# facebookresearch/detectron2

Measured on NVIDIA H100. Metric: Mask R-CNN R50-FPN training hot-path images/sec (custom-op path fwd+bwd, 2 images/GPU), higher is better.
Workload: dtype f32

## Files before the change

detectron2_b200/csrc/deform_conv_tc.cu:

```cuda
#include <algorithm>
#include <cstdlib>
#include <type_traits>

#include "common.cuh"
#include "deform_conv_tc.cuh"
#include "tc_common.cuh"

using namespace d2b_tc;

namespace {

constexpr int kWorkerWarps = 16;
constexpr int kWorkers = kWorkerWarps * 32;
constexpr int kThreads = kWorkers + 128;
constexpr int kLaunchRegs = (65536 / kThreads) & ~7;
constexpr int kWorkerRegs = 112, kSideRegs = 24;
static_assert(kWorkers * kWorkerRegs + (kThreads - kWorkers) * kSideRegs <= kThreads * kLaunchRegs,
              "register budget exceeds the launch allocation");
constexpr int kMaxBN = 128;
constexpr int kRowsPerHalf = 128 / (2 * kWorkerWarps);
constexpr int kTile = 16384;
constexpr int kMaxSmem = 227 * 1024;
constexpr int kGcolPitch = 132;

struct TC {
  int N, Cin, H, W, Cout, kh, kw, sh, sw, ph, pw, dh, dw, G, DG, Ho, Wo, cpg, opg, cpdg, KK, HoWo;
  int pack, SG, cps, ops, cbs, U;
  int tiles_img;
  int stages_img;
  int MC;
  int nks;
  long long off_bs, mask_bs;
  int mask_sigmoid;
};

struct Epi {
  const float* scale;
  const float* shift;
  int relu;
};

struct K1P { int BN, noct, goct, nkp, ksplit, S, tap_bytes, stage_bytes, red; };
struct K2P { int mper, msplit, tap_bytes; };
struct K3P { int BN, noct, sper, nsplit, S, stage_bytes; };

inline size_t align256(size_t v) { return (v + 255) & ~(size_t)255; }

bool make_tc(const d2b_dcn_params* p, TC& d) {
  if (!p) return false;
  d.N = p->N; d.Cin = p->Cin; d.H = p->H; d.W = p->W; d.Cout = p->Cout; d.kh = p->kh; d.kw = p->kw;
  d.sh = p->stride_h; d.sw = p->stride_w; d.ph = p->pad_h; d.pw = p->pad_w; d.dh = p->dil_h; d.dw = p->dil_w;
  d.G = p->groups; d.DG = p->deformable_groups;
  if (d.N < 0 || d.Cin <= 0 || d.H <= 0 || d.W <= 0 || d.Cout <= 0 || d.kh <= 0 || d.kw <= 0 || d.sh <= 0 || d.sw <= 0 ||
      d.ph < 0 || d.pw < 0 || d.dh <= 0 || d.dw <= 0 || d.G <= 0 || d.DG <= 0)
    return false;
  if (d.Cin % d.G || d.Cout % d.G || d.Cin % d.DG) return false;
  d.Ho = (d.H + 2 * d.ph - (d.dh * (d.kh - 1) + 1)) / d.sh + 1;
  d.Wo = (d.W + 2 * d.pw - (d.dw * (d.kw - 1) + 1)) / d.sw + 1;
  if (d.Ho <= 0 || d.Wo <= 0) return false;
  d.cpg = d.Cin / d.G; d.opg = d.Cout / d.G; d.cpdg = d.Cin / d.DG; d.KK = d.kh * d.kw; d.HoWo = d.Ho * d.Wo;
  if (d.cpg >= 64) {
    if (d.cpg % 64) return false;
    d.pack = 1;
  } else {
    if (d.cpg != 16 && d.cpg != 32) return false;
    d.pack = 64 / d.cpg;
    if (d.G % d.pack) return false;
  }
  if (d.cpdg % 64) return false;
  d.SG = d.G / d.pack; d.cps = d.cpg * d.pack; d.ops = d.opg * d.pack; d.cbs = d.cps / 64; d.U = d.KK * d.cbs;
  if (d.ops % 16) return false;
  if (d.KK > 49) return false;
  if ((long long)d.H * d.W * d.Cin >= (1LL << 29)) return false;
  if ((long long)d.HoWo * d.Cout >= (1LL << 31) || (long long)d.Cout * d.cpg * d.KK >= (1LL << 31)) return false;
  d.tiles_img = d2b_cdiv(d.HoWo, 128);
  d.stages_img = d2b_cdiv(d.HoWo, 64);
  d.MC = (d.U + 1) / 2;
  d.nks = d.ops / 64;
  if ((long long)d.N * d.tiles_img > 0x7fffffffLL) return false;
  d.off_bs = (long long)d.DG * 2 * d.KK * d.HoWo;
  d.mask_bs = (long long)d.DG * d.KK * d.HoWo;
  d.mask_sigmoid = 0;
  return true;
}

const float* use_fused_offset_mask(TC& d, const float* offset_mask) {
  d.off_bs = d.mask_bs = (long long)d.DG * 3 * d.KK * d.HoWo;
  d.mask_sigmoid = 1;
  return offset_mask + (size_t)d.DG * 2 * d.KK * d.HoWo;
}

int largest_tile(int n) {
  for (int t = kMaxBN; t >= 16; t >>= 1)
    if (n % t == 0) return t;
  return 0;
}

int best_split(long long base, int work, int max_split, int overhead) {
  int best = 1;
  long long best_cost = -1;
  for (int s = 1; s <= max_split; ++s) {
    const int per = d2b_cdiv(work, s);
    const int parts = d2b_cdiv(work, per);
    const long long cost = (long long)d2b_cdiv(base * parts, d2b_num_sms()) * (per + overhead);
    if (best_cost < 0 || cost < best_cost) {
      best_cost = cost;
      best = parts;
    }
  }
  return best;
}

bool plan_k1(const TC& d, K1P& k, bool colfed = false) {
  k.BN = largest_tile(d.ops);
  if (k.BN < 16) return false;
  k.noct = d.ops / k.BN;
  k.goct = colfed ? 1 : k.noct;
  const int base = d.N * d.tiles_img * d.SG * k.goct;
  k.ksplit = best_split(base, d.KK, d.KK, 1);
  k.nkp = d2b_cdiv(d.KK, k.ksplit);
  k.ksplit = d2b_cdiv(d.KK, k.nkp);
  k.red = k.ksplit > 1;
  const int ndg = d.DG == 1 ? 1 : std::min(d.DG, d2b_cdiv(d.cps, d.cpdg) + 1);
  k.tap_bytes = ndg * k.nkp * 128 * 16;
  k.stage_bytes = 2 * kTile + 2 * k.BN * 128;
  k.S = 3;
  while (k.S > 1 && k.S * k.stage_bytes + k.tap_bytes + 1024 + 128 > kMaxSmem) --k.S;
  return k.S >= 2;
}

bool plan_k1c(const TC& d, K1P& k1, K1P& kc) {
  const long long base = (long long)d.N * d.tiles_img * d.SG * (k1.noct - 1);
  if (k1.goct != 1 || k1.noct < 2 || (long long)d.N * d.tiles_img * (k1.noct - 1) > 0x7fffffffLL) return false;
  kc = k1;
  kc.goct = k1.noct - 1;
  kc.ksplit = best_split(base, d.KK, d.KK, 1);
  kc.nkp = d2b_cdiv(d.KK, kc.ksplit);
  kc.ksplit = d2b_cdiv(d.KK, kc.nkp);
  kc.tap_bytes = 0;
  kc.S = 3;
  while (kc.S > 1 && kc.S * kc.stage_bytes + 1024 + 128 > kMaxSmem) --kc.S;
  if (kc.S < 2) return false;
  k1.red = kc.red = k1.ksplit > 1 || kc.ksplit > 1;
  return true;
}

bool plan_k2(const TC& d, K2P& k) {
  if (d.ops % 64) return false;
  const int base = d.N * d.tiles_img * d.SG;
  k.msplit = best_split(base, d.MC, d.MC, 1);
  k.mper = d2b_cdiv(d.MC, k.msplit);
  k.msplit = d2b_cdiv(d.MC, k.mper);
  const int nkp = std::min(d.KK, (2 * k.mper + d.cbs - 1) / d.cbs + 1);
  const int ndg = d.DG == 1 ? 1 : std::min(d.DG, d2b_cdiv(d.cps, d.cpdg) + 1);
  k.tap_bytes = ndg * nkp * 128 * 16;
  return 2 * 4 * kTile + 128 * kGcolPitch * 4 + k.tap_bytes + 1024 + 128 <= kMaxSmem;
}

bool plan_k3(const TC& d, K3P& k) {
  if (d.ops % 64) return false;
  k.BN = largest_tile(d.ops);
  k.noct = d.ops / k.BN;
  const int units = d.MC * d.SG * k.noct;
  const int total = d.N * d.stages_img;
  k.nsplit = best_split(units, total, std::min(total, 4 * d2b_num_sms()), 3);
  k.sper = d2b_cdiv(total, k.nsplit);
  k.nsplit = d2b_cdiv(total, k.sper);
  k.stage_bytes = 2 * kTile + 2 * k.BN * 128;
  k.S = 3;
  while (k.S > 1 && k.S * k.stage_bytes + 4096 + 1024 + 128 > kMaxSmem) --k.S;
  return k.S >= 2;
}

struct Carve {
  size_t total = 0;
  size_t add(size_t bytes) {
    const size_t at = total;
    total += align256(bytes);
    return at;
  }
};

struct FwdPlan {
  TC d;
  K1P k1, kc;
  bool colfed;
  int split;
  size_t wt, x, total;
  size_t cols_bytes;
};

bool plan_fwd(const d2b_dcn_params* p, int precision, int x_nhwc, bool cols, FwdPlan& P) {
  if (!make_tc(p, P.d) || !plan_k1(P.d, P.k1)) return false;
  const TC& d = P.d;
  Carve ws;
  P.wt = ws.add((size_t)d.SG * P.k1.noct * d.U * 2 * P.k1.BN * 128);
  P.x = ws.add(x_nhwc ? 0 : sizeof(float) * (size_t)d.N * d.H * d.W * d.Cin);
  P.total = ws.total;
  P.cols_bytes = (size_t)d.N * d.tiles_img * d.SG * d.U * (size_t)(precision == 1 ? 2 : 1) * kTile;
  P.split = precision == 1 ? 1 : 0;
  P.colfed = false;
  K1P k1;
  if (cols && P.k1.noct > 1 && plan_k1(d, k1, true) && plan_k1c(d, k1, P.kc)) {
    P.k1 = k1;
    P.colfed = true;
  }
  return true;
}

struct BwdPlan {
  TC d;
  K2P k2;
  K3P k3;
  int split;
  size_t x, gx, gt_px, wt, gt_oc, gw, gw_bytes, total;
};

bool plan_bwd(const d2b_dcn_params* p, int precision, int x_nhwc, int need_data, int need_weight, BwdPlan& P) {
  if (!make_tc(p, P.d) || !plan_k2(P.d, P.k2) || !plan_k3(P.d, P.k3)) return false;
  const TC& d = P.d;
  const size_t xbytes = sizeof(float) * (size_t)d.N * d.H * d.W * d.Cin;
  P.gw_bytes = sizeof(float) * (size_t)d.SG * d.MC * 128 * d.ops;
  Carve ws;
  P.x = ws.add(x_nhwc ? 0 : xbytes);
  P.gx = ws.add(need_data && !x_nhwc ? xbytes : 0);
  P.gt_px = ws.add(need_data ? (size_t)d.N * d.tiles_img * d.SG * d.nks * 2 * kTile : 0);
  P.wt = ws.add(need_data ? (size_t)d.SG * d.MC * d.nks * 2 * kTile : 0);
  P.gt_oc = ws.add(need_weight ? (size_t)d.N * d.stages_img * d.SG * P.k3.noct * 2 * P.k3.BN * 128 : 0);
  P.gw = ws.add(need_weight ? P.gw_bytes : 0);
  P.total = ws.total;
  P.split = precision == 1 ? 1 : 0;
  return true;
}

struct TapRaw {
  float oh, ow, m;
};

__device__ __forceinline__ TapRaw tap_loads(const TC& d, const float* __restrict__ offset, const float* __restrict__ mask,
                                            int b, int dg, int kp, int p) {
  TapRaw r = {0.f, 0.f, 1.f};
  if (p < d.HoWo) {
    const size_t ob = (size_t)b * d.off_bs + ((size_t)dg * 2 * d.KK) * d.HoWo;
    r.oh = __ldg(offset + ob + (size_t)(2 * kp) * d.HoWo + p);
    r.ow = __ldg(offset + ob + (size_t)(2 * kp + 1) * d.HoWo + p);
    if (mask) r.m = __ldg(mask + (size_t)b * d.mask_bs + ((size_t)dg * d.KK + kp) * d.HoWo + p);
  }
  return r;
}

__device__ __forceinline__ int4 tap_finish(const TC& d, const TapRaw& r, bool has_mask, int kp, int p) {
  int4 t = make_int4(0, 0, 0, 0);
  if (p < d.HoWo) {
    const int ho = p / d.Wo, wo = p - ho * d.Wo;
    const int ki = kp / d.kw, kj = kp - ki * d.kw;
    const float hf = (float)(ho * d.sh - d.ph + ki * d.dh) + r.oh;
    const float wf = (float)(wo * d.sw - d.pw + kj * d.dw) + r.ow;
    float m = r.m;
    if (has_mask && d.mask_sigmoid) m = 1.f / (1.f + expf(-m));
    if (hf > -1.f && wf > -1.f && hf < (float)d.H && wf < (float)d.W) {
      const float hfl = floorf(hf), wfl = floorf(wf);
      const int hl = (int)hfl, wl = (int)wfl;
      const bool t0 = hl >= 0, t1 = hl + 1 <= d.H - 1, l0 = wl >= 0, l1 = wl + 1 <= d.W - 1;
      const int flags = (t0 && l0 ? 1 : 0) | (t0 && l1 ? 2 : 0) | (t1 && l0 ? 4 : 0) | (t1 && l1 ? 8 : 0);
      t.x = ((hl * d.W + wl + d.W + 1) << 4) | flags;
      t.y = __float_as_int(hf - hfl);
      t.z = __float_as_int(wf - wfl);
      t.w = __float_as_int(m);
    }
  }
  return t;
}

__device__ __forceinline__ int4 make_tap(const TC& d, const float* __restrict__ offset, const float* __restrict__ mask,
                                         int b, int dg, int kp, int p) {
  return tap_finish(d, tap_loads(d, offset, mask, b, dg, kp, p), mask != nullptr, kp, p);
}

struct Taps4 {
  float4 v0, v1, v2, v3;
};

__device__ __forceinline__ void load_corners(const float* __restrict__ xcb, uint32_t Cin, uint32_t rs, int code, Taps4& t) {
  const float* __restrict__ p = xcb + (uint32_t)(code >> 4) * Cin;
  const float4 z = make_float4(0.f, 0.f, 0.f, 0.f);
  t.v0 = (code & 1) ? __ldg(reinterpret_cast<const float4*>(p)) : z;
  t.v1 = (code & 2) ? __ldg(reinterpret_cast<const float4*>(p + Cin)) : z;
  t.v2 = (code & 4) ? __ldg(reinterpret_cast<const float4*>(p + rs)) : z;
  t.v3 = (code & 8) ? __ldg(reinterpret_cast<const float4*>(p + (rs + Cin))) : z;
}

__device__ __forceinline__ void interp4(const Taps4& t, float w0, float w1, float w2, float w3, float (&v)[4]) {
  const F2 z = f2_pack(0.f, 0.f), p0 = f2_pack(w0, w0), p1 = f2_pack(w1, w1), p2 = f2_pack(w2, w2), p3 = f2_pack(w3, w3);
  F2 a = f2_fma(p0, f2_pack(t.v0.x, t.v0.y), z), b = f2_fma(p0, f2_pack(t.v0.z, t.v0.w), z);
  a = f2_fma(p1, f2_pack(t.v1.x, t.v1.y), a);
  b = f2_fma(p1, f2_pack(t.v1.z, t.v1.w), b);
  a = f2_fma(p2, f2_pack(t.v2.x, t.v2.y), a);
  b = f2_fma(p2, f2_pack(t.v2.z, t.v2.w), b);
  a = f2_fma(p3, f2_pack(t.v3.x, t.v3.y), a);
  b = f2_fma(p3, f2_pack(t.v3.z, t.v3.w), b);
  f2_unpack(a, v[0], v[1]);
  f2_unpack(b, v[2], v[3]);
}

__device__ __forceinline__ void gather_store(const Taps4& t, int4 tap, uint8_t* a_hi, uint8_t* a_lo, uint32_t off,
                                             bool split) {
  const float lh = __int_as_float(tap.y), lw = __int_as_float(tap.z), m = __int_as_float(tap.w);
  const float hh = 1.f - lh, hw = 1.f - lw;
  float v[4];
// ... 99 lines not shown
    }
  }
  __syncthreads();
  if (warp < kWorkerWarps) reg_alloc<kWorkerRegs>();
  else reg_dealloc<kSideRegs>();

  if (warp < kWorkerWarps) {
    const int half = lane >> 4, q = lane & 15;
    const float* __restrict__ ximg = xh + (size_t)b * d.H * d.W * d.Cin - (size_t)(d.W + 1) * d.Cin;
    const uint32_t ucin = (uint32_t)d.Cin, urs = (uint32_t)(d.W * d.Cin);
    float acc[BN / 4];
#pragma unroll
    for (int i = 0; i < BN / 4; ++i) acc[i] = 0.f;
    int kpl = 0, cb = 0;
    auto stage = [&](int t) {
      const int s = t % k.S;
      const uint32_t par = (uint32_t)((t / k.S) & 1);
      const int cbase = sg * d.cps + cb * 64;
      const int4* __restrict__ tp = taps + ((cbase / d.cpdg - dg0) * nkp + kpl) * 128;
      const float* __restrict__ xc = ximg + cbase + q * 4;
      uint8_t* a_hi = smem + s * k.stage_bytes;
      uint8_t* a_lo = a_hi + kTile;
      mbar_wait(&empty_bar[s], par ^ 1u);
      {
        int4 tap[kRowsPerHalf];
        Taps4 c[kRowsPerHalf];
#pragma unroll
        for (int j = 0; j < kRowsPerHalf; ++j) tap[j] = tp[warp * 2 * kRowsPerHalf + j * 2 + half];
#pragma unroll
        for (int j = 0; j < kRowsPerHalf; ++j) load_corners(xc, ucin, urs, tap[j].x, c[j]);
#pragma unroll
        for (int j = 0; j < kRowsPerHalf; ++j) {
          const uint32_t r = (uint32_t)(warp * 2 * kRowsPerHalf + j * 2 + half);
          gather_store(c[j], tap[j], a_hi, a_lo, swz128(r, (uint32_t)(q >> 1)) + (uint32_t)(q & 1) * 8u, split != 0);
        }
      }
      fence_proxy_async();
      __syncwarp();
      if (lane == 0) mbar_arrive(&full_bar[s]);
      mbar_wait(&full_bar[s], par);
      const uint32_t sa = smem_u32(a_hi), sb = sa + 2 * kTile;
      mma_stage<BN, 0>(acc, sa, sa + kTile, sb, sb + (uint32_t)BN * 128u, split);
      if (++cb == d.cbs) { cb = 0; ++kpl; }
    };
    stage(0);
    for (int t = 1; t < nt; ++t) {
      stage(t);
      wgmma_wait<1>();
      __syncwarp();
      if (lane == 0) mbar_arrive(&empty_bar[(t - 1) % k.S]);
    }
    wgmma_wait<0>();
    fwd_epilogue<BN>(acc, ep, d, k, out, b, p0, sg * d.ops + oct * k.BN);
  } else if (warp == kWorkerWarps) {
    if (lane == 0) {
      const uint32_t bytes = (uint32_t)(split ? 2 : 1) * (uint32_t)k.BN * 128u;
      for (int t = 0; t < nt; ++t) {
        const int s = t % k.S;
        const uint32_t par = (uint32_t)((t / k.S) & 1);
        mbar_wait(&empty_bar[s], par ^ 1u);
        const size_t tile = ((size_t)(sg * k.noct + oct) * d.U + (size_t)kp0 * d.cbs + t);
        mbar_arrive_expect_tx(&full_bar[s], bytes);
        bulk_g2s(smem + s * k.stage_bytes + 2 * kTile, wt + tile * (size_t)(2 * k.BN * 128), bytes, &full_bar[s]);
      }
    }
  } else if (warp == kWorkerWarps + 1) {
    if (saving && lane == 0) {
      const uint32_t tile_bytes = (uint32_t)(split ? 2 : 1) * (uint32_t)kTile;
      for (int t = 0; t < nt; ++t) {
        const int s = t % k.S;
        const uint32_t par = (uint32_t)((t / k.S) & 1);
        mbar_wait(&full_bar[s], par);
        const size_t tile = ((size_t)blockIdx.x * d.SG + sg) * d.U + (size_t)kp0 * d.cbs + t;
        bulk_s2g(cols + tile * tile_bytes, smem + s * k.stage_bytes, tile_bytes);
        bulk_commit();
        bulk_wait_read0();
        mbar_arrive(&empty_bar[s]);
      }
      bulk_wait0();
    }
  }
}

template <int BN>
__global__ void __launch_bounds__(kThreads, 1) dcn_fwd_cols_kernel(const uint8_t* __restrict__ cols,
                                                                   const uint8_t* __restrict__ wt, const Epi ep, const TC d,
                                                                   const K1P k, const int split, float* __restrict__ out) {
  extern __shared__ uint8_t smem_raw[];
  uint8_t* smem = smem_raw + ((1024u - (smem_u32(smem_raw) & 1023u)) & 1023u);
  uint64_t* bars = reinterpret_cast<uint64_t*>(smem + k.S * k.stage_bytes);
  uint64_t* full_bar = bars;
  uint64_t* empty_bar = bars + k.S;

  const int tid = threadIdx.x, warp = tid >> 5, lane = tid & 31;
  const int tile = blockIdx.x / k.goct, oct = 1 + (blockIdx.x - tile * k.goct);
  const int b = tile / d.tiles_img, p0 = (tile - b * d.tiles_img) * 128;
  const int sg = blockIdx.y;
  const int kp0 = blockIdx.z * k.nkp, nkp = min(d.KK, kp0 + k.nkp) - kp0;
  const int nt = nkp * d.cbs;

  if (tid == 0) {
    for (int s = 0; s < k.S; ++s) {
      mbar_init(&full_bar[s], 1);
      mbar_init(&empty_bar[s], kWorkerWarps);
    }
    mbar_init_fence();
  }
  __syncthreads();
  if (warp < kWorkerWarps) reg_alloc<kWorkerRegs>();
  else reg_dealloc<kSideRegs>();

  if (warp < kWorkerWarps) {
    float acc[BN / 4];
#pragma unroll
    for (int i = 0; i < BN / 4; ++i) acc[i] = 0.f;
    auto issue = [&](int t) {
      const int s = t % k.S;
      mbar_wait(&full_bar[s], (uint32_t)((t / k.S) & 1));
      const uint32_t sa = smem_u32(smem + s * k.stage_bytes), sb = sa + 2 * kTile;
      mma_stage<BN, 0>(acc, sa, sa + kTile, sb, sb + (uint32_t)BN * 128u, split);
    };
    issue(0);
    for (int t = 1; t < nt; ++t) {
      issue(t);
      wgmma_wait<1>();
      __syncwarp();
      if (lane == 0) mbar_arrive(&empty_bar[(t - 1) % k.S]);
    }
    wgmma_wait<0>();
    fwd_epilogue<BN>(acc, ep, d, k, out, b, p0, sg * d.ops + oct * k.BN);
  } else if (warp == kWorkerWarps) {
    if (lane == 0) {
      const uint32_t parts = split ? 2u : 1u;
      const uint32_t abytes = parts * (uint32_t)kTile;
      const size_t u0 = (size_t)kp0 * d.cbs;
      const uint8_t* asrc = cols + (((size_t)tile * d.SG + sg) * d.U + u0) * abytes;
      const uint8_t* bsrc = wt + ((size_t)(sg * k.noct + oct) * d.U + u0) * (size_t)(2 * BN * 128);
      int s = 0;
      uint32_t par = 1u;
      for (int t = nt; t > 0; --t, asrc += abytes, bsrc += 2 * BN * 128) {
        mbar_wait(&empty_bar[s], par);
        mbar_arrive_expect_tx(&full_bar[s], abytes / 128u * (128u + BN));
        bulk_g2s(smem + s * k.stage_bytes, asrc, abytes, &full_bar[s]);
        bulk_g2s(smem + s * k.stage_bytes + 2 * kTile, bsrc, abytes / 128u * BN, &full_bar[s]);
        if (++s == k.S) {
          s = 0;
          par ^= 1u;
        }
      }
    }
  }
}

__global__ void __launch_bounds__(kThreads, 1) dcn_bwd_data_tc_kernel(const float* __restrict__ xh,
                                                                      const float* __restrict__ offset,
                                                                      const float* __restrict__ mask,
                                                                      const uint8_t* __restrict__ gt,
                                                                      const uint8_t* __restrict__ wt, const TC d,
                                                                      const K2P k, const int split,
                                                                      float* __restrict__ gxh, float* __restrict__ goff,
                                                                      float* __restrict__ gmask) {
  extern __shared__ uint8_t smem_raw[];
  uint8_t* smem = smem_raw + ((1024u - (smem_u32(smem_raw) & 1023u)) & 1023u);
  constexpr int kStage = 4 * kTile;
  float* gcol = reinterpret_cast<float*>(smem + 2 * kStage);
  int4* taps = reinterpret_cast<int4*>(smem + 2 * kStage + 128 * kGcolPitch * 4);
  uint64_t* bars = reinterpret_cast<uint64_t*>(reinterpret_cast<uint8_t*>(taps) + k.tap_bytes);
  uint64_t* full_bar = bars;
  uint64_t* empty_bar = bars + 2;

  const int tid = threadIdx.x, warp = tid >> 5, lane = tid & 31;
  const int b = blockIdx.x / d.tiles_img, pt = blockIdx.x - b * d.tiles_img, p0 = pt * 128;
  const int sg = blockIdx.y;
  const int m0 = blockIdx.z * k.mper, m1 = min(d.MC, m0 + k.mper), nm = m1 - m0;
  const int u_begin = 2 * m0, u_end = min(d.U, 2 * m1);
  const int kp0 = u_begin / d.cbs, nkp = (u_end - 1) / d.cbs - kp0 + 1;
  const int dg0 = (sg * d.cps) / d.cpdg;

  if (tid == 0) {
    for (int s = 0; s < 2; ++s) {
      mbar_init(&full_bar[s], 1);
      mbar_init(&empty_bar[s], kWorkerWarps);
    }
    mbar_init_fence();
  }
  if (tid < kWorkers) {
    const int ndg = ((sg + 1) * d.cps - 1) / d.cpdg - dg0 + 1;
    for (int i = tid; i < ndg * nkp * 128; i += kWorkers) {
      const int row = i & 127, r = i >> 7;
      const int dgl = r / nkp, kpl = r - dgl * nkp;
      taps[i] = make_tap(d, offset, mask, b, dg0 + dgl, kp0 + kpl, p0 + row);
    }
  }
  __syncthreads();
  if (warp < kWorkerWarps) reg_alloc<kWorkerRegs>();
  else reg_dealloc<kSideRegs>();

  if (warp < kWorkerWarps) {
    const int half = lane >> 4, q = lane & 15;
    const size_t img_off = (size_t)b * d.H * d.W * d.Cin - (size_t)(d.W + 1) * d.Cin;
    const float* __restrict__ ximg = xh + img_off;
    float* __restrict__ gimg = gxh ? gxh + img_off : nullptr;
    const uint32_t ucin = (uint32_t)d.Cin, urs = (uint32_t)(d.W * d.Cin);
    constexpr int R = kRowsPerHalf;
    float sh[R], sw[R], sm[R];
#pragma unroll
    for (int j = 0; j < R; ++j) sh[j] = sw[j] = sm[j] = 0.f;
    int cur_kp = -1, cur_dg = -1;

    auto flush = [&]() {
      if (cur_kp < 0) return;
      static_assert(R == 4, "the reduction below is written for 4 rows per half-warp");
      float v12[12];
#pragma unroll
      for (int j = 0; j < R; ++j) {
        v12[3 * j] = sh[j];
        v12[3 * j + 1] = sw[j];
        v12[3 * j + 2] = sm[j];
      }
      const bool b8 = q & 8, b4 = q & 4, b2 = q & 2, b1 = q & 1;
      float v6[6], v3[3];
#pragma unroll
      for (int i = 0; i < 6; ++i) {
        const float keep = b8 ? v12[i + 6] : v12[i], send = b8 ? v12[i] : v12[i + 6];
        v6[i] = keep + __shfl_xor_sync(0xffffffffu, send, 8);
      }
#pragma unroll
      for (int i = 0; i < 3; ++i) {
        const float keep = b4 ? v6[i + 3] : v6[i], send = b4 ? v6[i] : v6[i + 3];
        v3[i] = keep + __shfl_xor_sync(0xffffffffu, send, 4);
      }
      const float k0 = b2 ? v3[2] : v3[0], s0 = b2 ? v3[0] : v3[2];
      const float k1 = b2 ? 0.f : v3[1], s1 = b2 ? v3[1] : 0.f;
      const float u0 = k0 + __shfl_xor_sync(0xffffffffu, s0, 2);
      const float u1 = k1 + __shfl_xor_sync(0xffffffffu, s1, 2);
      float v = (b1 ? u1 : u0) + __shfl_xor_sync(0xffffffffu, b1 ? u0 : u1, 1);
      {
        const int j = q >> 2, which = q & 3;
        const int row = warp * 2 * R + j * 2 + half;
        const int p = p0 + row;
        if (which < 3 && p < d.HoWo) {
          if (which < 2) {
            if (goff) red_add(goff + (size_t)b * d.off_bs + ((size_t)cur_dg * 2 * d.KK + 2 * cur_kp + which) * d.HoWo + p, v);
          } else if (gmask) {
            if (d.mask_sigmoid) {
              const float m = __int_as_float(taps[((cur_dg - dg0) * nkp + (cur_kp - kp0)) * 128 + row].w);
              v *= m * (1.f - m);
            }
            red_add(gmask + (size_t)b * d.mask_bs + ((size_t)cur_dg * d.KK + cur_kp) * d.HoWo + p, v);
          }
        }
      }
#pragma unroll
      for (int j = 0; j < R; ++j) sh[j] = sw[j] = sm[j] = 0.f;
    };

    for (int ml = 0; ml < nm; ++ml) {
      const int buf = ml & 1;
      const int m = m0 + ml;
      const int nu = (2 * m + 1 < d.U) ? 2 : 1;
      {
        float acc[32];
#pragma unroll
        for (int i = 0; i < 32; ++i) acc[i] = 0.f;
        for (int ks = 0; ks < d.nks; ++ks) {
          const int c = ml * d.nks + ks, s = c & 1;
          mbar_wait(&full_bar[s], (uint32_t)((c >> 1) & 1));
          const uint32_t sa = smem_u32(smem + s * kStage);
          mma_stage<128, 0>(acc, sa, sa + kTile, sa + 2 * kTile, sa + 3 * kTile, split);
          wgmma_wait<0>();
          __syncwarp();
          if (lane == 0) mbar_arrive(&empty_bar[s]);
        }
#pragma unroll
        for (int i = 0; i < 32; i += 2)
          *reinterpret_cast<float2*>(gcol + acc_row<128>(i) * kGcolPitch + acc_col<128>(i)) = make_float2(acc[i], acc[i + 1]);
      }
      named_bar_sync(1, kWorkers);
      for (int ul = 0; ul < nu; ++ul) {
        const int u = 2 * m + ul;
        const int kp = u / d.cbs, cb = u - kp * d.cbs;
        const int cbase = sg * d.cps + cb * 64;
        const int dg = cbase / d.cpdg;
        if (kp != cur_kp || dg != cur_dg) {
          flush();
          cur_kp = kp;
          cur_dg = dg;
        }
        const int4* __restrict__ tp = taps + ((dg - dg0) * nkp + (kp - kp0)) * 128;
        const float* __restrict__ xc = ximg + cbase + q * 4;
        float* __restrict__ gc = gimg + cbase + q * 4;
        constexpr int kB2 = 2;
#pragma unroll
        for (int it = 0; it < R / kB2; ++it) {
          int4 tap[kB2];
          Taps4 c[kB2];
#pragma unroll
          for (int e = 0; e < kB2; ++e) tap[e] = tp[warp * 2 * R + (it * kB2 + e) * 2 + half];
#pragma unroll
          for (int e = 0; e < kB2; ++e) load_corners(xc, ucin, urs, tap[e].x, c[e]);
#pragma unroll
          for (int e = 0; e < kB2; ++e) {
            if ((tap[e].x & 15) == 0) continue;
            const int j = it * kB2 + e;
            const int row = warp * 2 * R + j * 2 + half;
            const float4 g4 = *reinterpret_cast<const float4*>(gcol + row * kGcolPitch + ul * 64 + q * 4);
            const float lh = __int_as_float(tap[e].y), lw = __int_as_float(tap[e].z), mk = __int_as_float(tap[e].w);
            const float hh = 1.f - lh, hw = 1.f - lw;
            const float w0 = hh * hw, w1 = hh * lw, w2 = lh * hw, w3 = lh * lw;
            const F2 LH = f2_pack(lh, lh), LW = f2_pack(lw, lw), HH = f2_pack(hh, hh), HW = f2_pack(hw, hw);
            const F2 W0 = f2_pack(w0, w0), W1 = f2_pack(w1, w1), W2 = f2_pack(w2, w2), W3 = f2_pack(w3, w3);
            const F2 MK = f2_pack(mk, mk);
            const F2 G[2] = {f2_pack(g4.x, g4.y), f2_pack(g4.z, g4.w)};
            const F2 A0[2] = {f2_pack(c[e].v0.x, c[e].v0.y), f2_pack(c[e].v0.z, c[e].v0.w)};
            const F2 A1[2] = {f2_pack(c[e].v1.x, c[e].v1.y), f2_pack(c[e].v1.z, c[e].v1.w)};
            const F2 A2[2] = {f2_pack(c[e].v2.x, c[e].v2.y), f2_pack(c[e].v2.z, c[e].v2.w)};
            const F2 A3[2] = {f2_pack(c[e].v3.x, c[e].v3.y), f2_pack(c[e].v3.z, c[e].v3.w)};
            F2 GM[2];
            F2 th2 = f2_pack(0.f, 0.f), tw2 = th2, tm2 = th2;
#pragma unroll
            for (int i = 0; i < 2; ++i) {
              GM[i] = f2_mul(G[i], MK);
              const F2 dh = f2_fma(LW, f2_sub(A3[i], A1[i]), f2_mul(HW, f2_sub(A2[i], A0[i])));
              const F2 dw = f2_fma(LH, f2_sub(A3[i], A2[i]), f2_mul(HH, f2_sub(A1[i], A0[i])));
              const F2 val = f2_fma(W3, A3[i], f2_fma(W2, A2[i], f2_fma(W1, A1[i], f2_mul(W0, A0[i]))));
              th2 = f2_fma(GM[i], dh, th2);
              tw2 = f2_fma(GM[i], dw, tw2);
              tm2 = f2_fma(G[i], val, tm2);
            }
            {
              float e0, e1;
              f2_unpack(th2, e0, e1);
              sh[j] += e0 + e1;
              f2_unpack(tw2, e0, e1);
              sw[j] += e0 + e1;
              f2_unpack(tm2, e0, e1);
              sm[j] += e0 + e1;
            }
            if (gimg) {
              float* gp = gc + (uint32_t)(tap[e].x >> 4) * ucin;
              red_add_v4_if(tap[e].x & 1, gp, f2_mul(GM[0], W0), f2_mul(GM[1], W0));
              red_add_v4_if(tap[e].x & 2, gp + ucin, f2_mul(GM[0], W1), f2_mul(GM[1], W1));
              red_add_v4_if(tap[e].x & 4, gp + urs, f2_mul(GM[0], W2), f2_mul(GM[1], W2));
              red_add_v4_if(tap[e].x & 8, gp + (urs + ucin), f2_mul(GM[0], W3), f2_mul(GM[1], W3));
            }
          }
        }
      }
      named_bar_sync(1, kWorkers);
    }
    flush();
  } else if (warp == kWorkerWarps) {
    if (lane == 0) {
      const uint32_t half_bytes = (uint32_t)(split ? 2 : 1) * (uint32_t)kTile;
      int c = 0;
      for (int ml = 0; ml < nm; ++ml) {
        const int m = m0 + ml;
        for (int ks = 0; ks < d.nks; ++ks, ++c) {
          const int s = c & 1;
          const uint32_t par = (uint32_t)((c >> 1) & 1);
          mbar_wait(&empty_bar[s], par ^ 1u);
          mbar_arrive_expect_tx(&full_bar[s], 2 * half_bytes);
          const size_t atile = (((size_t)b * d.tiles_img + pt) * d.SG + sg) * d.nks + ks;
          const size_t btile = ((size_t)sg * d.MC + m) * d.nks + ks;
          bulk_g2s(smem + s * kStage, gt + atile * (size_t)(2 * kTile), half_bytes, &full_bar[s]);
          bulk_g2s(smem + s * kStage + 2 * kTile, wt + btile * (size_t)(2 * kTile), half_bytes, &full_bar[s]);
        }
      }
    }
  }
}

template <int BN>
__device__ __forceinline__ void gw_tile_store(const float (&acc)[BN / 4], float* __restrict__ tile, int pitch) {
#pragma unroll
  for (int i = 0; i < BN / 4; i += 2) red_add_v2(tile + (size_t)acc_row<BN>(i) * pitch + acc_col<BN>(i), acc[i], acc[i + 1]);
}

__global__ void dcn_gw_reduce_kernel(const float* __restrict__ part, const TC d, float* __restrict__ gw) {
  const long long total = (long long)d.SG * d.U * 64 * d.ops;
  const long long idx = (long long)blockIdx.x * blockDim.x + threadIdx.x;
  if (idx >= total) return;
  const int ocl = (int)(idx % d.ops);
  const long long r = idx / d.ops;
  const int rowu = (int)(r % ((long long)d.U * 64)), sg = (int)(r / ((long long)d.U * 64));
  const int u = rowu >> 6, ch = rowu & 63;
  const int kp = u / d.cbs, cb = u - kp * d.cbs;
  const int ec = sg * d.cps + cb * 64 + ch, egrp = ec / d.cpg, ecin = ec - egrp * d.cpg;
  const int oc = sg * d.ops + ocl;
  if (oc / d.opg != egrp) return;
  gw[((size_t)oc * d.cpg + ecin) * d.KK + kp] = __ldg(part + ((size_t)sg * d.MC * 128 + rowu) * d.ops + ocl);
}

constexpr int kRedOc = 16, kRedCh = 16;
__global__ void __launch_bounds__(256) dcn_gw_reduce_tile_kernel(const float* __restrict__ part, const TC d,
                                                                  float* __restrict__ gw) {
  __shared__ float tile[9 * kRedCh][kRedOc + 1];
  const int per_sg = d.cps / kRedCh;
  const int sg = blockIdx.x / per_sg, c0 = (blockIdx.x - sg * per_sg) * kRedCh;
  const int cb = c0 >> 6, ch0 = c0 & 63;
  const int ocl0 = blockIdx.y * kRedOc;
  const int tid = threadIdx.x;
  {
    const int j = tid & (kRedOc - 1), r0 = tid / kRedOc;
    for (int row = r0; row < d.KK * kRedCh; row += 256 / kRedOc) {
      const int kp = row / kRedCh, ch = row - kp * kRedCh;
      tile[row][j] = __ldg(part + ((size_t)sg * d.MC * 128 + (size_t)(kp * d.cbs + cb) * 64 + ch0 + ch) * d.ops + ocl0 + j);
    }
  }
  __syncthreads();
  const int ec0 = sg * d.cps + c0;
  for (int i = tid; i < kRedOc * kRedCh * d.KK; i += 256) {
    const int j = i / (kRedCh * d.KK), e = i - j * (kRedCh * d.KK);
    const int ch = e / d.KK, kp = e - ch * d.KK;
    const int oc = sg * d.ops + ocl0 + j, grp = oc / d.opg;
    const int ec = ec0 + ch;
    if (ec / d.cpg == grp) gw[((size_t)oc * d.cpg + (ec - grp * d.cpg)) * d.KK + kp] = tile[kp * kRedCh + ch][j];
  }
}

template <int BN>
__global__ void __launch_bounds__(kThreads, 1) dcn_bwd_weight_tc_kernel(const float* __restrict__ xh,
                                                                        const float* __restrict__ offset,
                                                                        const float* __restrict__ mask,
                                                                        const uint8_t* __restrict__ gt, const TC d,
                                                                        const K3P k, const int split,
                                                                        float* __restrict__ gw) {
  extern __shared__ uint8_t smem_raw[];
  uint8_t* smem = smem_raw + ((1024u - (smem_u32(smem_raw) & 1023u)) & 1023u);
  int4* tap_s = reinterpret_cast<int4*>(smem + k.S * k.stage_bytes);
  uint64_t* bars = reinterpret_cast<uint64_t*>(reinterpret_cast<uint8_t*>(tap_s) + 4096);
  uint64_t* full_bar = bars;
  uint64_t* empty_bar = bars + k.S;

  const int tid = threadIdx.x, warp = tid >> 5, lane = tid & 31;
  const int mb = blockIdx.y;
  const int sg = blockIdx.x / k.noct, oct = blockIdx.x - sg * k.noct;
  const int total = d.N * d.stages_img;
  const int gs0 = blockIdx.z * k.sper, gs1 = min(total, gs0 + k.sper), ns = gs1 - gs0;

  if (tid == 0) {
    for (int s = 0; s < k.S; ++s) {
      mbar_init(&full_bar[s], kWorkerWarps + 1);
      mbar_init(&empty_bar[s], kWorkerWarps);
    }
    mbar_init_fence();
  }
  __syncthreads();
  if (warp < kWorkerWarps) reg_alloc<kWorkerRegs>();
  else reg_dealloc<kSideRegs>();

  if (warp < kWorkerWarps) {
    const int half = lane >> 4, q = lane & 15;
    const int u = 2 * mb + half;
    const bool u_ok = u < d.U;
    const int kp = u_ok ? u / d.cbs : 0, cb = u_ok ? u - kp * d.cbs : 0;
    const int cbase = sg * d.cps + cb * 64;
    const int dg = cbase / d.cpdg;
    constexpr int PX = 64 / kWorkerWarps;
    const int tl_half = (lane / PX) & 1, tl_j = lane % PX;
    const int tl_u = 2 * mb + tl_half;
    const bool tl_ok = lane < 2 * PX && tl_u < d.U;
    const int tl_kp = tl_ok ? tl_u / d.cbs : 0;
    const int tl_dg = tl_ok ? (sg * d.cps + (tl_u - tl_kp * d.cbs) * 64) / d.cpdg : 0;
    int4* my_taps = tap_s + warp * 2 * (2 * PX);
    auto stage_of = [&](int i, int& b, int& pbase) {
      const int gs = gs0 + i;
      b = gs / d.stages_img;
      pbase = (gs - b * d.stages_img) * 64;
    };
    if (ns > 0) {
      int b0, pb0;
      stage_of(0, b0, pb0);
      if (lane < 2 * PX) my_taps[lane] = tl_ok ? make_tap(d, offset, mask, b0, tl_dg, tl_kp, pb0 + warp * PX + tl_j) : make_int4(0, 0, 0, 0);
    }
    __syncwarp();
    float acc[BN / 4];
#pragma unroll
    for (int i = 0; i < BN / 4; ++i) acc[i] = 0.f;
    auto stage = [&](int i) {
      const int s = i % k.S;
      const uint32_t par = (uint32_t)((i / k.S) & 1);
      int b, pbase, bn = 0, pbn = 0;
      stage_of(i, b, pbase);
      const bool have_next = i + 1 < ns;
      TapRaw raw = {0.f, 0.f, 1.f};
      if (have_next) {
        stage_of(i + 1, bn, pbn);
        if (tl_ok) raw = tap_loads(d, offset, mask, bn, tl_dg, tl_kp, pbn + warp * PX + tl_j);
      }
      const float* __restrict__ xc = xh + ((size_t)b * d.H * d.W - (size_t)(d.W + 1)) * d.Cin + cbase + q * 4;
      const uint32_t ucin = (uint32_t)d.Cin, urs = (uint32_t)(d.W * d.Cin);
      uint8_t* a_hi = smem + s * k.stage_bytes + half * 8192;
      uint8_t* a_lo = a_hi + kTile;
      const int4* cur = my_taps + (i & 1) * (2 * PX) + half * PX;
      mbar_wait(&empty_bar[s], par ^ 1u);
      {
        int4 tap[PX];
        Taps4 c[PX];
#pragma unroll
        for (int j = 0; j < PX; ++j) tap[j] = cur[j];
#pragma unroll
        for (int j = 0; j < PX; ++j) load_corners(xc, ucin, urs, tap[j].x, c[j]);
#pragma unroll
        for (int j = 0; j < PX; ++j) {
          const uint32_t r = (uint32_t)(warp * PX + j);
          gather_store(c[j], tap[j], a_hi, a_lo, swz128(r, (uint32_t)(q >> 1)) + (uint32_t)(q & 1) * 8u, split != 0);
        }
      }
      if (have_next && lane < 2 * PX)
        my_taps[((i + 1) & 1) * (2 * PX) + lane] =
            tl_ok ? tap_finish(d, raw, mask != nullptr, tl_kp, pbn + warp * PX + tl_j) : make_int4(0, 0, 0, 0);
      fence_proxy_async();
      __syncwarp();
      if (lane == 0) mbar_arrive(&full_bar[s]);
      mbar_wait(&full_bar[s], par);
      const uint32_t sa = smem_u32(smem + s * k.stage_bytes), sb = sa + 2 * kTile;
      mma_stage<BN, 1>(acc, sa, sa + kTile, sb, sb + (uint32_t)BN * 128u, split);
    };
// ... 281 lines not shown
  D2B_CHECK_LAUNCH();
  return D2B_OK;
}

template <int W, int... More, class Launch>
int with_tile_width(int BN, Launch launch) {
  if constexpr (sizeof...(More) > 0)
    if (BN != W) return with_tile_width<More...>(BN, launch);
  return launch(std::integral_constant<int, W>());
}

}

D2B_API int d2b_deform_conv_tc_shape_supported(const d2b_dcn_params* p, int backward) {
  FwdPlan f;
  BwdPlan b;
  return backward ? plan_bwd(p, 1, 1, 1, 1, b) : plan_fwd(p, 1, 1, false, f);
}

size_t d2b_deform_conv_tc_fwd_workspace(const d2b_dcn_params* p, int precision, int x_nhwc) {
  FwdPlan P;
  return plan_fwd(p, precision, x_nhwc, false, P) ? P.total : 0;
}

size_t d2b_deform_conv_tc_bwd_workspace(const d2b_dcn_params* p, int precision, int x_nhwc, int need_data, int need_weight) {
  BwdPlan P;
  return plan_bwd(p, precision, x_nhwc, need_data, need_weight, P) ? P.total : 0;
}

size_t d2b_deform_conv_tc_cols_bytes(const d2b_dcn_params* p, int precision) {
  FwdPlan f;
  BwdPlan b;
  return plan_fwd(p, precision, 1, false, f) && plan_bwd(p, precision, 1, 0, 0, b) ? f.cols_bytes : 0;
}

int d2b_deform_conv_forward_tc(const float* x, const float* offset, const float* mask, const float* weight,
                               const float* scale, const float* shift, int relu, const d2b_dcn_params* p, int precision,
                               int tcflags, float* out, void* cols, void* workspace, size_t workspace_bytes, void* stream_) {
  cudaStream_t stream = (cudaStream_t)stream_;
  const int x_nhwc = tcflags & 1;
  FwdPlan P;
  if (!plan_fwd(p, precision, x_nhwc, cols != nullptr, P)) return D2B_EUNSUPPORTED;
  TC& d = P.d;
  const K1P& k = P.k1;
  if (d.N == 0) return D2B_OK;
  if (tcflags & 2) {
    if (mask) return D2B_EINVAL;
    mask = use_fused_offset_mask(d, offset);
  }
  if (!workspace || workspace_bytes < P.total) return D2B_EWORKSPACE;
  if ((reinterpret_cast<uintptr_t>(workspace) & 255) || (x_nhwc && (reinterpret_cast<uintptr_t>(x) & 15)) ||
      (reinterpret_cast<uintptr_t>(cols) & 15))
    return D2B_EINVAL;
  uint8_t* ws = reinterpret_cast<uint8_t*>(workspace);
  uint8_t* wt = ws + P.wt;
  const float* xh = x;
  if (!x_nhwc) {
    float* xn = reinterpret_cast<float*>(ws + P.x);
    if (int rc = change_layout(x, d, xn, true, stream)) return rc;
    xh = xn;
  }
  {
    const long long total = (long long)d.SG * k.noct * d.U * k.BN * 8;
    dcn_wtile_fwd_kernel<<<d2b_cdiv(total, 256), 256, 0, stream>>>(weight, d, k.BN, k.noct, wt);
    D2B_CHECK_LAUNCH();
  }
  if (k.red) D2B_CUDA(cudaMemsetAsync(out, 0, sizeof(float) * (size_t)d.N * d.Cout * d.HoWo, stream));
  const Epi ep = {scale, shift, relu};
  const dim3 grid(d.N * d.tiles_img, d.SG * k.goct, k.ksplit);
  const int smem_bytes = k.S * k.stage_bytes + k.tap_bytes + 1024 + 128;
  int rc = with_tile_width<16, 32, 64, 128>(k.BN, [&](auto bn) {
    return launch_big_smem<dcn_fwd_tc_kernel<decltype(bn)::value>>(grid, smem_bytes, stream, xh, offset, mask, wt, ep, d, k,
                                                                    P.split, out, reinterpret_cast<uint8_t*>(cols));
  });
  if (rc) return rc;
  if (P.colfed) {
    const K1P& kc = P.kc;
    const dim3 grid_c(d.N * d.tiles_img * kc.goct, d.SG, kc.ksplit);
    const int smem_c = kc.S * kc.stage_bytes + 1024 + 128;
    const uint8_t* cl = reinterpret_cast<const uint8_t*>(cols);
    rc = with_tile_width<16, 32, 64, 128>(kc.BN, [&](auto bn) {
      return launch_big_smem<dcn_fwd_cols_kernel<decltype(bn)::value>>(grid_c, smem_c, stream, cl, wt, ep, d, kc, P.split,
                                                                        out);
    });
    if (rc) return rc;
  }
  if (k.red && (scale || relu)) {
    const long long total = (long long)d.N * d.Cout * d.HoWo;
    dcn_epilogue_kernel<<<d2b_cdiv(total, 256), 256, 0, stream>>>(out, total, d.Cout, d.HoWo, ep);
    D2B_CHECK_LAUNCH();
  }
  return D2B_OK;
}

int d2b_deform_conv_backward_tc(const float* x, const float* offset, const float* mask, const float* weight,
                                const float* grad_out, const float* scale, const float* y_saved, int relu,
                                const d2b_dcn_params* p, int precision, int tcflags, const void* cols, float* grad_x,
                                float* grad_offset, float* grad_mask, float* grad_weight, void* workspace,
                                size_t workspace_bytes, void* stream_) {
  cudaStream_t stream = (cudaStream_t)stream_;
  const int x_nhwc = tcflags & 1;
  const int need_data = (grad_x || grad_offset || grad_mask) ? 1 : 0, need_weight = grad_weight ? 1 : 0;
  BwdPlan P;
  if (!plan_bwd(p, precision, x_nhwc, need_data, need_weight, P)) return D2B_EUNSUPPORTED;
  TC& d = P.d;
  const K2P& k2 = P.k2;
  const K3P& k3 = P.k3;
  const bool fused_om = (tcflags & 2) != 0;
  if (fused_om && (mask || grad_mask)) return D2B_EINVAL;
  if (relu && !y_saved) return D2B_EINVAL;
  const size_t nx = (size_t)d.N * d.H * d.W * d.Cin, noff = (size_t)d.N * d.DG * (fused_om ? 3 : 2) * d.KK * d.HoWo;
  const size_t nm = (size_t)d.N * d.DG * d.KK * d.HoWo, nw = (size_t)d.Cout * d.cpg * d.KK;
  if (fused_om) {
    mask = use_fused_offset_mask(d, offset);
    if (grad_offset) grad_mask = grad_offset + (size_t)d.DG * 2 * d.KK * d.HoWo;
  }
  const Epi ep = {scale, nullptr, relu};
  if (d.N == 0 || (!need_data && !need_weight)) {
    void* zp[3] = {grad_offset, fused_om ? nullptr : grad_mask, grad_weight};
    size_t zb[3] = {noff * 4, nm * 4, nw * 4};
    return d2b_zero_buffers(zp, zb, 3, stream);
  }
  if (!workspace || workspace_bytes < P.total) return D2B_EWORKSPACE;
  if ((reinterpret_cast<uintptr_t>(workspace) & 255) || (x_nhwc && (reinterpret_cast<uintptr_t>(x) & 15)) ||
      (x_nhwc && grad_x && (reinterpret_cast<uintptr_t>(grad_x) & 15)) || (reinterpret_cast<uintptr_t>(cols) & 15))
    return D2B_EINVAL;
  uint8_t* ws = reinterpret_cast<uint8_t*>(workspace);
  const float* xh = x;
  if (!x_nhwc) {
    float* xn = reinterpret_cast<float*>(ws + P.x);
    if (int rc = change_layout(x, d, xn, true, stream)) return rc;
    xh = xn;
  }
  float* gxh = grad_x ? (x_nhwc ? grad_x : reinterpret_cast<float*>(ws + P.gx)) : nullptr;
  uint8_t* gt_oc = need_weight ? ws + P.gt_oc : nullptr;
  float* gw_part = need_weight ? reinterpret_cast<float*>(ws + P.gw) : nullptr;
  {
    void* zp[4] = {grad_offset, fused_om ? nullptr : grad_mask, gxh, gw_part};
    size_t zb[4] = {noff * 4, nm * 4, nx * 4, P.gw_bytes};
    int rc = d2b_zero_buffers(zp, zb, 4, stream);
    if (rc) return rc;
  }
  if (need_data) {
    uint8_t* gt_px = ws + P.gt_px;
    uint8_t* wt = ws + P.wt;
    dcn_gout_px_tiles_kernel<<<dim3((unsigned)((size_t)d.N * d.tiles_img * d.SG * d.nks), 4), 256, 0, stream>>>(
        grad_out, y_saved, ep, d, gt_px, gt_oc, k3.BN, k3.noct);
    D2B_CHECK_LAUNCH();
    {
      const long long total = (long long)d.SG * d.MC * d.nks * 128 * 8;
      dcn_wtile_bwd_kernel<<<d2b_cdiv(total, 256), 256, 0, stream>>>(weight, d, wt);
      D2B_CHECK_LAUNCH();
    }
    const int smem_bytes = 2 * 4 * kTile + 128 * kGcolPitch * 4 + k2.tap_bytes + 1024 + 128;
    if (int rc = launch_big_smem<dcn_bwd_data_tc_kernel>(dim3(d.N * d.tiles_img, d.SG, k2.msplit), smem_bytes, stream, xh,
                                                         offset, mask, gt_px, wt, d, k2, P.split, gxh, grad_offset,
                                                         mask ? grad_mask : nullptr))
      return rc;
    if (grad_x && !x_nhwc) {
      if (int rc = change_layout(gxh, d, grad_x, false, stream)) return rc;
    }
  }
  if (need_weight) {
    if (!need_data) {
      const long long total = (long long)d.N * d.stages_img * d.SG * k3.noct * k3.BN * 8;
      dcn_gout_oc_tiles_kernel<<<d2b_cdiv(total, 256), 256, 0, stream>>>(grad_out, y_saved, ep, d, k3.BN, k3.noct, gt_oc);
      D2B_CHECK_LAUNCH();
    }
    const dim3 grid(d.SG * k3.noct, d.MC, k3.nsplit);
    int rc;
    if (cols) {
      const int S = std::min(6, (kMaxSmem - 2048) / k3.stage_bytes);
      const int smem_bytes = S * k3.stage_bytes + 1024 + 128;
      const uint8_t* cl = reinterpret_cast<const uint8_t*>(cols);
      rc = with_tile_width<64, 128>(k3.BN, [&](auto bn) {
        return launch_big_smem<dcn_bwd_weight_cols_kernel<decltype(bn)::value>>(grid, smem_bytes, stream, cl, gt_oc, d, k3, S,
                                                                                 P.split, gw_part);
      });
    } else {
      const int smem_bytes = k3.S * k3.stage_bytes + 4096 + 1024 + 128;
      rc = with_tile_width<64, 128>(k3.BN, [&](auto bn) {
        return launch_big_smem<dcn_bwd_weight_tc_kernel<decltype(bn)::value>>(grid, smem_bytes, stream, xh, offset, mask, gt_oc,
                                                                               d, k3, P.split, gw_part);
      });
    }
    if (rc) return rc;
    if (d.KK <= 9) {
      dcn_gw_reduce_tile_kernel<<<dim3(d.SG * (d.cps / kRedCh), d.ops / kRedOc), 256, 0, stream>>>(gw_part, d, grad_weight);
    } else {
      const long long total = (long long)d.SG * d.U * 64 * d.ops;
      dcn_gw_reduce_kernel<<<d2b_cdiv(total, 256), 256, 0, stream>>>(gw_part, d, grad_weight);
    }
    D2B_CHECK_LAUNCH();
  }
  return D2B_OK;
}
```

Measured before the change: 284.8.

## Pipeline deformable-conv backward-data kernel with three smem slots and in-place gcol

Replaces the separate padded gcol buffer plus double-buffered stages with three TMA stage slots. The last stage's slot is reused for the swizzled gcol tile and released to the producer only after the scatter phase, behind an async-proxy fence. The wgmma loop now keeps one group in flight with wait<1> and releases the previous slot. The bilinear scatter loop also software-prefetches taps and corners two rows ahead. The aim is to overlap TMA loads, MMA and scatter work and to cut shared-memory bank conflicts, at the cost of trickier slot and phase bookkeeping and more register pressure.

```diff
diff --git a/detectron2_b200/csrc/deform_conv_tc.cu b/detectron2_b200/csrc/deform_conv_tc.cu
--- a/detectron2_b200/csrc/deform_conv_tc.cu
+++ b/detectron2_b200/csrc/deform_conv_tc.cu
@@ -21,7 +21,7 @@
 constexpr int kRowsPerHalf = 128 / (2 * kWorkerWarps);
 constexpr int kTile = 16384;
 constexpr int kMaxSmem = 227 * 1024;
-constexpr int kGcolPitch = 132;
+constexpr int kK2Stage = 4 * kTile, kK2Slots = 3;
 
 struct TC {
   int N, Cin, H, W, Cout, kh, kw, sh, sw, ph, pw, dh, dw, G, DG, Ho, Wo, cpg, opg, cpdg, KK, HoWo;
@@ -154,7 +154,7 @@
   const int nkp = std::min(d.KK, (2 * k.mper + d.cbs - 1) / d.cbs + 1);
   const int ndg = d.DG == 1 ? 1 : std::min(d.DG, d2b_cdiv(d.cps, d.cpdg) + 1);
   k.tap_bytes = ndg * nkp * 128 * 16;
-  return 2 * 4 * kTile + 128 * kGcolPitch * 4 + k.tap_bytes + 1024 + 128 <= kMaxSmem;
+  return kK2Slots * kK2Stage + k.tap_bytes + 1024 + 128 <= kMaxSmem;
 }
 
 bool plan_k3(const TC& d, K3P& k) {
@@ -560,6 +560,11 @@
   }
 }
 
+
+__device__ __forceinline__ uint32_t gcol_off(uint32_t row, uint32_t col) {
+  return row * 512u + ((((col >> 2) ^ ((row & 3u) << 1))) << 4) + (col & 3u) * 4u;
+}
+
 __global__ void __launch_bounds__(kThreads, 1) dcn_bwd_data_tc_kernel(const float* __restrict__ xh,
                                                                       const float* __restrict__ offset,
                                                                       const float* __restrict__ mask,
@@ -570,12 +575,11 @@
                                                                       float* __restrict__ gmask) {
   extern __shared__ uint8_t smem_raw[];
   uint8_t* smem = smem_raw + ((1024u - (smem_u32(smem_raw) & 1023u)) & 1023u);
-  constexpr int kStage = 4 * kTile;
-  float* gcol = reinterpret_cast<float*>(smem + 2 * kStage);
-  int4* taps = reinterpret_cast<int4*>(smem + 2 * kStage + 128 * kGcolPitch * 4);
+  constexpr int S = kK2Slots;
+  int4* taps = reinterpret_cast<int4*>(smem + S * kK2Stage);
   uint64_t* bars = reinterpret_cast<uint64_t*>(reinterpret_cast<uint8_t*>(taps) + k.tap_bytes);
   uint64_t* full_bar = bars;
-  uint64_t* empty_bar = bars + 2;
+  uint64_t* empty_bar = bars + S;
 
   const int tid = threadIdx.x, warp = tid >> 5, lane = tid & 31;
   const int b = blockIdx.x / d.tiles_img, pt = blockIdx.x - b * d.tiles_img, p0 = pt * 128;
@@ -586,7 +590,7 @@
   const int dg0 = (sg * d.cps) / d.cpdg;
 
   if (tid == 0) {
-    for (int s = 0; s < 2; ++s) {
+    for (int s = 0; s < S; ++s) {
       mbar_init(&full_bar[s], 1);
       mbar_init(&empty_bar[s], kWorkerWarps);
     }
@@ -606,6 +610,10 @@
 
   if (warp < kWorkerWarps) {
     const int half = lane >> 4, q = lane & 15;
+    auto release = [&](int c) {
+      __syncwarp();
+      if (lane == 0) mbar_arrive(&empty_bar[c % S]);
+    };
     const size_t img_off = (size_t)b * d.H * d.W * d.Cin - (size_t)(d.W + 1) * d.Cin;
     const float* __restrict__ ximg = xh + img_off;
     float* __restrict__ gimg = gxh ? gxh + img_off : nullptr;
@@ -664,25 +672,31 @@
     };
 
     for (int ml = 0; ml < nm; ++ml) {
-      const int buf = ml & 1;
       const int m = m0 + ml;
       const int nu = (2 * m + 1 < d.U) ? 2 : 1;
+      const int c0 = ml * d.nks, clast = c0 + d.nks - 1;
+      uint8_t* gcol = smem + (clast % S) * kK2Stage;
       {
         float acc[32];
 #pragma unroll
         for (int i = 0; i < 32; ++i) acc[i] = 0.f;
-        for (int ks = 0; ks < d.nks; ++ks) {
-          const int c = ml * d.nks + ks, s = c & 1;
-          mbar_wait(&full_bar[s], (uint32_t)((c >> 1) & 1));
-          const uint32_t sa = smem_u32(smem + s * kStage);
+        auto issue = [&](int c) {
+          const int s = c % S;
+          mbar_wait(&full_bar[s], (uint32_t)((c / S) & 1));
+          const uint32_t sa = smem_u32(smem + s * kK2Stage);
           mma_stage<128, 0>(acc, sa, sa + kTile, sa + 2 * kTile, sa + 3 * kTile, split);
-          wgmma_wait<0>();
-          __syncwarp();
-          if (lane == 0) mbar_arrive(&empty_bar[s]);
+        };
+        issue(c0);
+        for (int c = c0 + 1; c <= clast; ++c) {
+          issue(c);
+          wgmma_wait<1>();
+          release(c - 1);
         }
+        wgmma_wait<0>();
+        named_bar_sync(1, kWorkers);
 #pragma unroll
         for (int i = 0; i < 32; i += 2)
-          *reinterpret_cast<float2*>(gcol + acc_row<128>(i) * kGcolPitch + acc_col<128>(i)) = make_float2(acc[i], acc[i + 1]);
+          *reinterpret_cast<float2*>(gcol + gcol_off(acc_row<128>(i), acc_col<128>(i))) = make_float2(acc[i], acc[i + 1]);
       }
       named_bar_sync(1, kWorkers);
       for (int ul = 0; ul < nu; ++ul) {
@@ -698,21 +712,19 @@
         const int4* __restrict__ tp = taps + ((dg - dg0) * nkp + (kp - kp0)) * 128;
         const float* __restrict__ xc = ximg + cbase + q * 4;
         float* __restrict__ gc = gimg + cbase + q * 4;
-        constexpr int kB2 = 2;
-#pragma unroll
-        for (int it = 0; it < R / kB2; ++it) {
-          int4 tap[kB2];
-          Taps4 c[kB2];
-#pragma unroll
-          for (int e = 0; e < kB2; ++e) tap[e] = tp[warp * 2 * R + (it * kB2 + e) * 2 + half];
-#pragma unroll
-          for (int e = 0; e < kB2; ++e) load_corners(xc, ucin, urs, tap[e].x, c[e]);
-#pragma unroll
-          for (int e = 0; e < kB2; ++e) {
-            if ((tap[e].x & 15) == 0) continue;
-            const int j = it * kB2 + e;
+        int4 tap[2];
+        Taps4 c[2];
+#pragma unroll
+        for (int e = 0; e < 2; ++e) {
+          tap[e] = tp[warp * 2 * R + e * 2 + half];
+          load_corners(xc, ucin, urs, tap[e].x, c[e]);
+        }
+#pragma unroll
+        for (int j = 0; j < R; ++j) {
+          const int e = j & 1;
+          if (tap[e].x & 15) {
             const int row = warp * 2 * R + j * 2 + half;
-            const float4 g4 = *reinterpret_cast<const float4*>(gcol + row * kGcolPitch + ul * 64 + q * 4);
+            const float4 g4 = *reinterpret_cast<const float4*>(gcol + gcol_off(row, ul * 64 + q * 4));
             const float lh = __int_as_float(tap[e].y), lw = __int_as_float(tap[e].z), mk = __int_as_float(tap[e].w);
             const float hh = 1.f - lh, hw = 1.f - lw;
             const float w0 = hh * hw, w1 = hh * lw, w2 = lh * hw, w3 = lh * lw;
@@ -753,9 +765,14 @@
               red_add_v4_if(tap[e].x & 8, gp + (urs + ucin), f2_mul(GM[0], W3), f2_mul(GM[1], W3));
             }
           }
+          if (j + 2 < R) {
+            tap[e] = tp[warp * 2 * R + (j + 2) * 2 + half];
+            load_corners(xc, ucin, urs, tap[e].x, c[e]);
+          }
         }
       }
-      named_bar_sync(1, kWorkers);
+      fence_proxy_async();
+      release(clast);
     }
     flush();
   } else if (warp == kWorkerWarps) {
@@ -765,14 +782,14 @@
       for (int ml = 0; ml < nm; ++ml) {
         const int m = m0 + ml;
         for (int ks = 0; ks < d.nks; ++ks, ++c) {
-          const int s = c & 1;
-          const uint32_t par = (uint32_t)((c >> 1) & 1);
+          const int s = c % S;
+          const uint32_t par = (uint32_t)((c / S) & 1);
           mbar_wait(&empty_bar[s], par ^ 1u);
           mbar_arrive_expect_tx(&full_bar[s], 2 * half_bytes);
           const size_t atile = (((size_t)b * d.tiles_img + pt) * d.SG + sg) * d.nks + ks;
           const size_t btile = ((size_t)sg * d.MC + m) * d.nks + ks;
-          bulk_g2s(smem + s * kStage, gt + atile * (size_t)(2 * kTile), half_bytes, &full_bar[s]);
-          bulk_g2s(smem + s * kStage + 2 * kTile, wt + btile * (size_t)(2 * kTile), half_bytes, &full_bar[s]);
+          bulk_g2s(smem + s * kK2Stage, gt + atile * (size_t)(2 * kTile), half_bytes, &full_bar[s]);
+          bulk_g2s(smem + s * kK2Stage + 2 * kTile, wt + btile * (size_t)(2 * kTile), half_bytes, &full_bar[s]);
         }
       }
     }
@@ -1360,7 +1377,7 @@
       dcn_wtile_bwd_kernel<<<d2b_cdiv(total, 256), 256, 0, stream>>>(weight, d, wt);
       D2B_CHECK_LAUNCH();
     }
-    const int smem_bytes = 2 * 4 * kTile + 128 * kGcolPitch * 4 + k2.tap_bytes + 1024 + 128;
+    const int smem_bytes = kK2Slots * kK2Stage + k2.tap_bytes + 1024 + 128;
     if (int rc = launch_big_smem<dcn_bwd_data_tc_kernel>(dim3(d.N * d.tiles_img, d.SG, k2.msplit), smem_bytes, stream, xh,
                                                          offset, mask, gt_px, wt, d, k2, P.split, gxh, grad_offset,
                                                          mask ? grad_mask : nullptr))
```

Result: no change. 287.5 (median of 6 runs) (+1.0%).
